# latk/hbetune.rs

Hardware: AMD Instinct MI355X
Metric: GP fit+predict/sec (n=4096,d=8,f64) (higher is better)
Workload: dtype f64; 1 GPU; M: rosenbrock d=8 n=4096 f64, Matern nu=5/2 x constant + white noise; fixed-work fit = 3 L-BFGS runs x 150 lml+gradient evaluations + K^-1, then predict mean+variance at m=1600; evals_per_fit=450, n_not_pd=0, m_candidates=1600, parallelism=replicas x1 (independent fits per GPU, no collective)

## Files before the change

csrc/dag_plan.hpp:

```cpp
#pragma once
#include <algorithm>
#include <cstdint>
#include <cstdio>
#include <queue>
#include <string>
#include <vector>

#include "engine.hpp"

namespace hbegp {

inline int dag_split_point(int lo, int hi) { return lo + (hi - lo) / 2; }

struct DagPlan {
  std::vector<DagTask> tasks;
  std::vector<int> totals;
  double gflop = 0;
  double gflop_lauum = 0;
  int n_lauum = 0;
  int n_leaf = 0;
  double sim_us = 0;
  double crit_us = 0;
};

struct DagGate {
  int cnt = -1, val = 0;
};

struct DagCosts {
  double leaf = 28.5 + 4.0;
  double overhead = 1.5 + 4.0;
  double per128_big = 7.9;
  double per128_small = 3.9;
  double per128_big128 = 15.0;
  double per128_chain = 1.5;
};

class DagBuilder {
 public:
  DagBuilder(int bk, int small_h, int nwg = 0, bool fine = true) : bk_(bk), small_h_(small_h), nwg_(nwg), fine_(fine) {}

  void set_rl(int group, int near, bool lauum_split = true, bool chain32 = true) {
    rl_group_ = std::max(1, group); rl_near_ = std::max(1, near); rl_lauum_split_ = lauum_split; rl_chain32_ = chain32;
  }
  void set_rl_progressive(bool on) { rl_prog_ = on; }
  DagPlan build(int blo, int bhi, bool lauum = false, bool rl = false) {
    plan_ = DagPlan();
    top_lo_ = blo; top_hi_ = bhi;
    if (rl && blo == 0) {
      lauum_split_ = rl_lauum_split_;
      build_rl(bhi, lauum);
    } else {
      const Sub root = rec(blo, bhi, nullptr);
      if (lauum && blo == 0) build_lauum(bhi, root);
    }
    if (plan_.totals.size() >= 0xffff) plan_.tasks.clear();
    for (int tot : plan_.totals)
      if (tot > 0xffff) plan_.tasks.clear();
    if (nwg_ > 0 && !plan_.tasks.empty()) order();
    return plan_;
  }

 private:
  static constexpr int crit_rows_ = 1;
  int bk_, small_h_, nwg_;
  bool fine_;
  int rl_group_ = 32, rl_near_ = 1;
  bool rl_lauum_split_ = true;
  bool big128_ = false;
  bool big128_acc_ = false;
  bool rl_prog_ = false;
  bool rl_chain32_ = true;
  DagPlan plan_;
  DagCosts cost_;

  int new_counter() {
    plan_.totals.push_back(0);
    return (int)plan_.totals.size() - 1;
  }
  void push(DagTask t, const std::vector<DagGate>& waits, int sig0, int sig1, double cost_us, int sig2 = -1) {
// ... 91 lines not shown
      std::stable_sort(tiles.begin() + row_begin, tiles.end(), [](const Tile& a, const Tile& b) {
        auto wt = [](int kind) { return kind == DAG_GEMM_128x128 ? 4 : (kind == DAG_GEMM_128x64 ? 2 : 1); };
        const long wa = (long)(a.kb - a.ka) * wt(a.kind), wb = (long)(b.kb - b.ka) * wt(b.kind);
        return wa > wb;
      });
    }
    return tiles;
  }
  DagTask make(const Op& op, const Tile& tl, double* cost_us) {
    DagTask t{};
    t.kind = (uint16_t)tl.kind;
    t.flags = op.flags;
    t.row0 = tl.row0; t.col0 = tl.col0;
    t.kbeg = tl.ka / bk_ * bk_;
    t.kend = (tl.kb + bk_ - 1) / bk_ * bk_;
    *cost_us = cost_.overhead + (t.kend - t.kbeg) / 128.0 * (tl.kind == DAG_GEMM_128x128 ? cost_.per128_big128 : (tl.kind == DAG_GEMM_128x64 ? cost_.per128_big : (tl.kind == DAG_GEMM_32x64 ? cost_.per128_chain : cost_.per128_small)));
    return t;
  }
  static int count_row(const std::vector<Tile>& tiles, int bi) {
    int c = 0;
    for (const Tile& t : tiles) c += t.bi == bi;
    return c;
  }

  int top_lo_ = 0, top_hi_ = 0, top_mid_ = -1;
  DagGate top_right_all_;
  DagGate top_left_all_;
  bool lauum_split_ = false;
  struct Sub {
    int lo = 0, hi = 0;
    std::vector<DagGate> rowfin;
    DagGate all;
  };
  typedef std::vector<DagGate> RowGates;

  Sub rec(int lo, int hi, const RowGates* gate) {
    Sub out;
    out.lo = lo; out.hi = hi;
    auto gate_of = [&](int i) { return (gate && i < (int)gate->size()) ? (*gate)[i] : DagGate(); };
    if (hi - lo == 1) {
      DagTask t{};
      t.kind = DAG_LEAF;
      t.row0 = lo;
      const int c = new_counter();
      push(t, {gate_of(lo)}, c, -1, cost_.leaf);
      plan_.n_leaf++;
      out.rowfin.assign(1, DagGate{c, 1});
      out.all = DagGate{c, 1};
      return out;
    }
    const int mid = dag_split_point(lo, hi);
    const bool small = std::max(mid - lo, hi - mid) <= small_h_;
    const Sub left = rec(lo, mid, gate);
    double cu = 0;
    Op t{};
    t.flags = DAGF_BBUF | DAGF_CBUF;
    t.r0 = mid; t.r1 = hi; t.c0 = lo; t.c1 = mid; t.k0 = lo; t.k1 = mid; t.klim = 1; t.tri_b = true; t.crit = 1;
    const std::vector<Tile> tt = tiles_of(t, small);
    RowGates trow(hi);
    for (int i = mid; i < hi; ++i) trow[i] = DagGate{new_counter(), count_row(tt, i)};
// ... 123 lines not shown
      stack.push_back({f.lo, mid});
      stack.push_back({mid, f.hi});
    }
    std::vector<DagGate> leafc(nb);
    std::vector<std::vector<DagGate>> lc(nb, std::vector<DagGate>(nb)), last_upd(nb, std::vector<DagGate>(nb));
    std::vector<std::vector<std::pair<int, int>>> groups(nb);
    for (int j = 0; j < nb; ++j) groups[j] = rl_groups(j, GROUP, NEAR);
    double cu = 0;
    auto single_tile = [&](Op op, int i, int j) { op.r0 = i; op.r1 = i + 1; op.c0 = j; op.c1 = j + 1; return op; };
    for (int k = 0; k < nb; ++k) {
      {
        DagTask t{};
        t.kind = DAG_LEAF;
        t.row0 = k;
        const int c = new_counter();
        push(t, {last_upd[k][k]}, c, -1, cost_.leaf);
        plan_.n_leaf++;
        leafc[k] = DagGate{c, 1};
      }
      for (int i = k + 1; i < nb; ++i) {
        Op t{};
        t.flags = DAGF_BBUF | DAGF_C3;
        t.k0 = k; t.k1 = k + 1; t.klim = 1; t.tri_b = true;
        const std::vector<Tile> tt = tiles_of(single_tile(t, i, k), i - k <= NEAR, rl_chain32_ && i == k + 1);
        const int c = new_counter();
        lc[i][k] = DagGate{c, (int)tt.size()};
        const int nd = node_of[i][k];
        for (const Tile& tl : tt) {
          const DagTask tk = make(t, tl, &cu);
          push(tk, {leafc[k], last_upd[i][k], k > 0 ? lc[i][k - 1] : DagGate()}, c, nodes[nd].lrow[i - nodes[nd].mid], cu);
        }
// ... 155 lines not shown
    const std::vector<Tile> xt = tiles_of(x, small);
    RowGates xrow(hi);
    for (int i = mid; i < hi; ++i) xrow[i] = DagGate{new_counter(), count_row(xt, i)};
    const DagGate xall{new_counter(), (int)xt.size()};
    for (const Tile& tl : xt) {
      const DagTask tk = make(x, tl, &cu);
      push(tk, {fine_ ? right.rowfin[tl.bi - mid] : right.all, uall}, xrow[tl.bi].cnt, xall.cnt, cu);
    }
    out.rowfin.resize(hi - lo);
    for (int j = lo; j < mid; ++j) out.rowfin[j - lo] = left.rowfin[j - lo];
    for (int j = mid; j < hi; ++j) out.rowfin[j - lo] = xrow[j];
    out.all = xall;
    return out;
  }

  void order() {
    const int nt = (int)plan_.tasks.size(), nc = (int)plan_.totals.size();
    std::vector<std::vector<int>> waiters(nc);
    for (int i = 0; i < nt; ++i)
      for (int w = 0; w < plan_.tasks[i].nwait; ++w) waiters[plan_.tasks[i].wcnt[w]].push_back(i);
    std::vector<double> bl(nt, 0.0), blc(nc, 0.0);
    for (int i = nt - 1; i >= 0; --i) {
      const DagTask& t = plan_.tasks[i];
      double tail = 0;
      for (int q = 0; q < DAG_MAXSIG; ++q)
        if (t.sig[q] != DAG_NOSIG) tail = std::max(tail, blc[t.sig[q]]);
      bl[i] = t.cost * 0.1 + tail;
      for (int w = 0; w < t.nwait; ++w) blc[t.wcnt[w]] = std::max(blc[t.wcnt[w]], bl[i]);
    }
    plan_.crit_us = *std::max_element(bl.begin(), bl.end());
    std::vector<int> count(nc, 0), missing(nt, 0);
    typedef std::pair<double, int> Pri;
    std::priority_queue<Pri> ready;
    for (int i = 0; i < nt; ++i) {
      missing[i] = plan_.tasks[i].nwait;
      if (missing[i] == 0) ready.push({bl[i], -i});
    }
    typedef std::pair<double, int> Ev;
    std::priority_queue<Ev, std::vector<Ev>, std::greater<Ev>> running;
    std::vector<DagTask> out;
    out.reserve(nt);
    std::vector<int> out_idx;
    std::vector<double> start(nt, 0.0);
    out_idx.reserve(nt);
    int idle = nwg_;
    double now = 0;
    while ((int)out.size() < nt) {
      while (idle > 0 && !ready.empty()) {
        const int i = -ready.top().second;
        ready.pop();
        out.push_back(plan_.tasks[i]);
        out_idx.push_back(i);
        start[i] = now;
        running.push({now + plan_.tasks[i].cost * 0.1, i});
        --idle;
      }
      if (running.empty()) break;
      const Ev e = running.top();
      running.pop();
      now = e.first;
// ... 40 lines not shown
    t.nwait = 0;
    for (int w = 0; w < DAG_MAXWAIT; ++w) t.wcnt[w] = t.wval[w] = 0;
    for (int w = 0; w < src.nwait; ++w) {
      if (remap[src.wcnt[w]] < 0) continue;
      t.wcnt[t.nwait] = (uint16_t)remap[src.wcnt[w]];
      t.wval[t.nwait] = src.wval[w];
      ++t.nwait;
    }
    out.tasks.push_back(t);
  }
  out.gflop = out.gflop_lauum = full.gflop_lauum;
  out.n_lauum = (int)out.tasks.size();
  out.sim_us = full.sim_us;
  out.crit_us = full.crit_us;
  return out;
}

inline std::string dag_plan_validate(const DagPlan& plan, int nblocks_total) {
  const int nc = (int)plan.totals.size(), nt = (int)plan.tasks.size();
  const int words = (nc + 63) / 64;
  char buf[256];
  std::vector<int> count(nc, 0);
  std::vector<uint64_t> counter_known((size_t)nc * words, 0), cur(words);
  const int nt64 = nblocks_total * 4;
  struct Cell { int writer = -1; std::vector<int> readers; };
  constexpr int NBUF = 8;
  std::vector<Cell> cells[NBUF];
  for (int b = 0; b < NBUF; ++b) cells[b].resize((size_t)nt64 * nt64);
  std::vector<std::vector<uint64_t>> known(nt);
  auto hb = [&](int a, int b) -> bool {
// ... 104 lines not shown
```

csrc/hbegp.cpp:

```cpp
#include "../include/hbegp.h"

#include <hip/hip_runtime_api.h>

#include <algorithm>
#include <atomic>
#include <queue>
#include <cmath>
#include <cstdarg>
#include <cstdio>
#include <cstdlib>
#include <cstring>
#include <functional>
#include <limits>
#include <memory>
#include <mutex>
#include <numeric>
#include <string>
#include <thread>
#include <type_traits>
#include <vector>

#include "dag_plan.hpp"
#include "engine.hpp"
#include "lbfgsb.hpp"
// ... 571 lines not shown
    (*off)[w] = (int)items->size();
    items->insert(items->end(), per[w].begin(), per[w].end());
  }
  (*off)[nwg] = (int)items->size();
  *nwg_out = nwg;
  return true;
}

constexpr int DAG_MAX_VARIANTS = 4;
constexpr int DAG_CROWD_LEVELS = 3;
constexpr int DAG_CROWD_BUSY[DAG_CROWD_LEVELS] = {6, 12, 24};
constexpr int DAG_SHARE_VARIANTS = 2;
constexpr int MAX_DEVS = 64;
struct DagPlanKey {
  int blocks, bk, small_h, nwg, lauum, rl, rl_group, rl_near, lauum_split, chain32, prog, big128;
  auto tie() const { return std::tie(blocks, bk, small_h, nwg, lauum, rl, rl_group, rl_near, lauum_split, chain32, prog, big128); }
  bool operator<(const DagPlanKey& o) const { return tie() < o.tie(); }
};
static std::atomic<int> g_dev_busy[MAX_DEVS];
static std::atomic<int> g_dev_fits[MAX_DEVS];

template <typename T>
struct LooIn {
  int dev;
  hipStream_t s;
  int n, d, np, nu2;
  const T *X, *y, *alpha, *Xinv, *Kinv;
  const EvalParams* P;
};
template <typename T>
static int loo_tail(const LooIn<T>& in, T* mean, T* var, T* lpd, double* loo, double* grad);

template <typename T>
struct Slot {
  int dev = 0;
  hipStream_t stream = nullptr;
  T *Xalt = nullptr, *ldalt = nullptr;
  bool x_captured = false;
  T *W1 = nullptr, *W2 = nullptr, *Kinv[2] = {nullptr, nullptr}, *alpha[2] = {nullptr, nullptr};
  T* W3 = nullptr;
  T *ldiag = nullptr, *wbuf = nullptr;
  double *part_t = nullptr, *part_g = nullptr;
  EvalParams* dP = nullptr;
  EvalOut* dOut = nullptr;
  int* tickets = nullptr;
  unsigned long long* dag_trace = nullptr;
  int* dag_ctrl = nullptr;
  EvalParams* hP = nullptr;
  EvalOut* hOut = nullptr;
  void* small_slab = nullptr;
  size_t small_slab_bytes = 0;
  void* host_slab = nullptr;
  size_t host_slab_bytes = 0;
  hipGraphExec_t graph[DAG_MAX_VARIANTS + 1 + DAG_CROWD_LEVELS + DAG_SHARE_VARIANTS][2][4] = {};
  int best_idx = -1;
  double best_lml = -std::numeric_limits<double>::infinity();
  int best_run = 0, best_eval = 0;
  std::vector<double> best_theta;
  std::vector<double> best_params;
  int last_target = 0;
  int dag_variant = 1;
// ... 43 lines not shown
  int dag_nshare_ = 0;
  int share_hyst_ = SLOT_SHARE_HYSTERESIS;
  int slot_maxeval_ = 0;
  std::vector<int> share_force_;
  std::vector<char> balance_dev_;
  std::unique_ptr<std::atomic<int>[]> slot_running_, slot_done_;
  mutable std::atomic<int> not_alone_{0};
  unsigned long long dag_wait_ticks_ = 200000000ull;
  size_t dag_ctrl_bytes = 0;
  int dag_ctrl_regions_ = 1;
  double dag_gflop = 0;
  bool adhoc_ = false;
  bool small_ = false;
  bool like_fit_ = false;
  bool lazy_ = false;
  std::function<std::shared_ptr<const DagPlan>(int, bool)> plan_for_;
  bool hostio_ = true;
  bool eval_published() const { return hostio_ && !small_; }
  int leaf_dbg_ = 0;

  struct Pooled { int dev; void* p; size_t bytes; };
  std::vector<Pooled> pooled_;
  template <typename U>
  U* palloc(int dev, size_t count) {
    bool fresh = false;
    const size_t bytes = std::max<size_t>(16, sizeof(U) * count);
    void* q = g_pool.get(dev, bytes, &fresh);
    pooled_.push_back({dev, q, bytes});
    return static_cast<U*>(q);
  }

// ... 87 lines not shown
      int cus = 1 << 30;
      for (int dev : c->devs) {
        hipDeviceProp_t prop;
        HIPCHECK(hipGetDeviceProperties(&prop, dev));
        cus = std::min(cus, std::max(1, prop.multiProcessorCount));
      }
      const int forced = env_int("HBEGP_DAG_WG", 0);
      auto share_of = [&](int busy) {
        const int share = busy <= 1 ? cus : std::max(8, (cus * 112 / 100 / busy + 4) / 8 * 8);
        return forced > 0 ? forced : std::max(1, std::min(cus, share));
      };
      dag_lauum_ = env_int("HBEGP_DAG_LAUUM", 1) != 0;
      dag_rl_ = env_int("HBEGP_DAG_RL", np / NB <= 80 ? 1 : 0) != 0;
      static std::mutex cache_mu;
      static std::map<DagPlanKey, std::shared_ptr<const DagPlan>> cache;
      plan_for_ = [this](int nwg, bool lauum) {
        const DagPlanKey key = {np / NB, dag_stage_depth(is_f32), env_int("HBEGP_DAG_SMALLH", dag_rl_ ? 4 : 8), nwg, lauum, dag_rl_,
                                env_int("HBEGP_DAG_RL_GROUP", 32), env_int("HBEGP_DAG_RL_NEAR", 1),
                                env_int("HBEGP_DAG_LAUUM_SPLIT", n_slots <= 1 ? 1 : 0),
                                env_int("HBEGP_DAG_CHAIN32", 1),
                                env_int("HBEGP_DAG_PROG", np / NB <= DAG_PROG_MAX_BLOCKS ? 1 : 0),
                                env_int("HBEGP_DAG_BIG128", ((n_slots >= 2 && np / NB >= 32) || np / NB >= 64) ? 2 : 0)};
        std::shared_ptr<const DagPlan> cached;
        {
          std::lock_guard<std::mutex> lk(cache_mu);
          auto it = cache.find(key);
          if (it != cache.end()) cached = it->second;
        }
        if (!cached) {
          DagBuilder builder(key.bk, key.small_h, key.nwg);
          builder.set_rl(key.rl_group, key.rl_near, key.lauum_split != 0, key.chain32 != 0);
          builder.set_rl_progressive(key.prog != 0);
          builder.set_big128(key.big128 != 0, key.big128 >= 2);
          cached = std::make_shared<const DagPlan>(builder.build(0, np / NB, lauum, dag_rl_));
          std::lock_guard<std::mutex> lk(cache_mu);
          if (cache.size() > 256) cache.clear();
          cache[key] = cached;
        }
        return cached;
      };
      const int nvar = std::min(n_slots, DAG_MAX_VARIANTS);
      dag_nwg = share_of(n_slots);
      auto plan_for = [this](int nwg) { return plan_for_(nwg, dag_lauum_); };
      std::shared_ptr<const DagPlan> cached = plan_for(dag_nwg);
      if (cached->tasks.empty() && dag_rl_) {
        dag_rl_ = false;
        cached = plan_for(dag_nwg);
      }
      const DagPlan& plan = *cached;
      if (plan.tasks.empty()) dag_ = dag_lauum_ = false;
      if (dag_ && env_int("HBEGP_DAG_VALIDATE", 0)) {
        const std::string why = dag_plan_validate(plan, np / NB);
        if (!why.empty()) throw std::runtime_error("task queue of the factorisation is unsound: " + why);
      }
      if (dag_) {
        dag_ntasks = (int)plan.tasks.size();
        dag_nwg = std::min(dag_nwg, dag_ntasks);
        dag_gflop = plan.gflop;
// ... 23 lines not shown
          share_force_.resize(n_slots, SLOT_SHARE_EVEN);
        }
        share_hyst_ = std::max(0, env_int("HBEGP_RUN_BALANCE_HYST", SLOT_SHARE_HYSTERESIS));
        dag_nshare_ = (adapt && n_slots > 1 && (env_int("HBEGP_RUN_BALANCE", np / NB >= SLOT_SHARE_MIN_BLOCKS ? 1 : 0) != 0 || !share_force_.empty())) ? DAG_SHARE_VARIANTS : 0;
        if (dag_nshare_) {
          balance_dev_.assign(c->devs.size(), 0);
          slot_running_.reset(new std::atomic<int>[c->devs.size() * n_slots]);
          slot_done_.reset(new std::atomic<int>[c->devs.size() * n_slots]);
          for (size_t i = 0; i < c->devs.size() * n_slots; ++i) { slot_running_[i].store(0); slot_done_[i].store(0); }
        }
        dag_var.assign(nvar + 1 + dag_ncrowd_ + dag_nshare_, DagVariant());
        for (int v = 1; v <= nvar + dag_ncrowd_ + dag_nshare_; ++v) {
          DagVariant& var = dag_var[v];
          std::shared_ptr<const DagPlan> pv = cached;
          var.nwg = dag_nwg;
          if (v != nvar && adapt) {
            if (v > nvar + dag_ncrowd_) {
              var.nwg = std::min(share_wg[v - nvar - dag_ncrowd_ - 1], dag_ntasks);
            } else {
              const int busy = v < nvar ? v : DAG_CROWD_BUSY[v - nvar - 1];
              var.nwg = std::min(share_of(busy), dag_ntasks);
              if (v > nvar) var.nwg = std::min(var.nwg, dag_nwg);
            }
            pv = plan_for(var.nwg);
            if (pv->tasks.size() != plan.tasks.size()) { pv = cached; var.nwg = dag_nwg; }
          }
          var.host_tasks = pv->tasks;
          var.tasks.assign(c->devs.size(), nullptr);
          for (size_t di = 0; di < c->devs.size(); ++di) {
            HIPCHECK(hipSetDevice(c->devs[di]));
            var.tasks[di] = palloc<DagTask>(c->devs[di], pv->tasks.size());
            HIPCHECK(hipMemcpyAsync(var.tasks[di], var.host_tasks.data(), sizeof(DagTask) * var.host_tasks.size(), hipMemcpyHostToDevice, slots[di][0].stream));
          }
          if (lazy_ && dag_lauum_) {
            const int wg_p1 = lazy_wg(var.nwg, 1), wg_kinv = lazy_wg(var.nwg, 2);
            const std::shared_ptr<const DagPlan> p1 = plan_for_(wg_p1, false);
            const DagPlan kv = dag_plan_kinv_only(*pv);
            if (p1->tasks.empty() || kv.tasks.empty() || p1->totals.size() > plan.totals.size() || kv.totals.size() > plan.totals.size()) {
              throw std::runtime_error("task queues of a two-phase evaluation could not be derived from the plan");
            } else {
              if (env_int("HBEGP_DAG_VALIDATE", 0)) {
                std::string why = dag_plan_validate(*p1, np / NB);
                if (why.empty()) why = dag_plan_validate(kv, np / NB);
                if (!why.empty()) throw std::runtime_error("task queue of a two-phase evaluation is unsound: " + why);
              }
              var.host_tasks_p1 = p1->tasks;
              var.host_tasks_kinv = kv.tasks;
              var.ntasks_p1 = (int)p1->tasks.size();
              var.ntasks_kinv = (int)kv.tasks.size();
              var.nwg_p1 = std::min(wg_p1, var.ntasks_p1);
              var.nwg_kinv = std::min(wg_kinv, var.ntasks_kinv);
              var.tasks_p1.assign(c->devs.size(), nullptr);
// ... 40 lines not shown
        if (build_sched(g, sc.tile, &off, &items, &nwg)) {
          sc.nwg = nwg;
          sc.d_off = palloc<int>(s.dev, off.size());
          sc.d_items = palloc<unsigned>(s.dev, items.size());
          HIPCHECK(hipMemcpyAsync(sc.d_off, off.data(), sizeof(int) * off.size(), hipMemcpyHostToDevice, s.stream));
          HIPCHECK(hipMemcpyAsync(sc.d_items, items.data(), sizeof(unsigned) * items.size(), hipMemcpyHostToDevice, s.stream));
          HIPCHECK(hipStreamSynchronize(s.stream));
        }
        scheds[di].push_back(sc);
      };
      eval_gemms(s, s.Kinv[0], record, [](int) {}, [] {});
    }
  }
  ~Problem() override { release(); }

  void release() {
    for (size_t di = 0; di < slots.size(); ++di) {
      (void)hipSetDevice(ctx->devs[di]);
      for (auto& s : slots[di]) {
        if (s.stream) (void)hipStreamSynchronize(s.stream);
        for (int v = 0; v <= DAG_MAX_VARIANTS + DAG_CROWD_LEVELS + DAG_SHARE_VARIANTS; ++v)
          for (int a = 0; a < 2; ++a)
            for (int b = 0; b < 4; ++b)
              if (s.graph[v][a][b]) (void)hipGraphExecDestroy(s.graph[v][a][b]);
        const size_t nnb = sizeof(T) * (size_t)np * np;
        g_pool.put(s.dev, s.W1, nnb); g_pool.put(s.dev, s.W2, nnb); g_pool.put(s.dev, s.W3, nnb);
        for (int b = 0; b < 2; ++b) g_pool.put(s.dev, s.Kinv[b], nnb);
        g_pool.put(s.dev, s.small_slab, s.small_slab_bytes);
        g_host_pool.put(s.host_slab, s.host_slab_bytes);
        g_stream_pool.put(s.dev, s.stream);
      }
// ... 359 lines not shown
          enqueue_eval(s, di, target, mode, nullptr);
        } catch (...) {
          (void)hipStreamEndCapture(s.stream, &gr);
          throw;
        }
        HIPCHECK(hipStreamEndCapture(s.stream, &gr));
        HIPCHECK(hipGraphInstantiate(&ge, gr, nullptr, nullptr, 0));
        HIPCHECK(hipGraphDestroy(gr));
      }
      HIPCHECK(hipGraphLaunch(ge, s.stream));
    } else {
      enqueue_eval(s, di, target, mode, nullptr);
    }
    s.published = eval_published();
    wait_eval(s, t_launch, mode);
    s.last_target = target;
    const int p = d + 2;
    if (s.hOut->info < 0) {
      dag_report_timeout(s);
      throw HipError{hipErrorLaunchTimeOut, "factorisation task queue: a dependency wait exceeded its bound", __LINE__};
    }
    if (s.hOut->info != 0) {
      if (mode != EVAL_GRAD_ONLY) *lml = -std::numeric_limits<double>::infinity();
      if (grad) for (int j = 0; j < p; ++j) grad[j] = 0.0;
      return HBEGP_NOT_PD;
    }
    double lml_kept = s.hOut->lml;
    if (mode == EVAL_GRAD_ONLY) lml = &lml_kept;
    if (!(s.hOut->done & 1) || (want_grad && !(s.hOut->done & 2)))
      throw HipError{hipErrorLaunchFailure, "evaluation: the lml/gradient kernels did not run", __LINE__};
// ... 3589 lines not shown
  DagPlan plan = builder.build(0, nblocks, which != 1, (fine & 8) != 0);
  if (which == 2) plan = dag_plan_kinv_only(plan);
  const std::string why = plan.tasks.empty() ? std::string("no tasks") : dag_plan_validate(plan, nblocks);
  *ntasks = (int)plan.tasks.size();
  if (tasks)
    for (int i = 0; i < std::min(cap, (int)plan.tasks.size()); ++i) {
      const DagTask& t = plan.tasks[i];
      const int v[6] = {t.kind, t.flags, t.row0, t.col0, t.kbeg, t.kend};
      memcpy(tasks + (size_t)6 * i, v, sizeof v);
    }
  if (err && errlen > 0) snprintf(err, (size_t)errlen, "%s", why.c_str());
  return why.empty() ? HBEGP_OK : fail(HBEGP_EINVAL, "%s", why.c_str());
  GUARD_END
}

int hbegp_debug_lbfgs_replay(int n, const double* x0, const double* lo, const double* hi, int maxeval, int memory, int fixed_work,
                             int count, const double* f, const double* g, double* requested, int* n_requested) {
  if (n < 1 || n > LBFGS_MAXN || count < 0 || !x0 || !lo || !hi || !requested || !n_requested || (count > 0 && (!f || !g)))
    return fail(HBEGP_EINVAL, "bad argument");
  GUARD_BEGIN
  return lbfgs_replay_impl(n, x0, lo, hi, maxeval, memory, fixed_work, count, f, g, requested, nullptr, nullptr, nullptr, n_requested);
  GUARD_END
}

int hbegp_debug_dag_plan(int nblocks, int bk, int small_h, int nwg, int fine, int* ntasks, int* ncounters, int* nleaf,
                         double* gflop, double* crit_us, double* sim_us, char* err, int errlen) {
  if (nblocks < 1 || (bk != 16 && bk != 32) || small_h < 0 || nwg < 0) return fail(HBEGP_EINVAL, "bad argument");
  GUARD_BEGIN
  DagBuilder builder(bk, small_h, nwg, (fine & 1) != 0);
  builder.set_rl_progressive((fine & 16) != 0);
// ... 48 lines not shown
```

hbetune_rs_amd/_lib.py:

```python
import ctypes as C
import os

import numpy as np

HERE = os.path.dirname(os.path.abspath(__file__))
LIB_PATH = os.environ.get("HBEGP_LIB") or os.path.join(HERE, "libhbegp.so")

OK, NOT_PD, ALL_FAILED = 0, 1, 2
EINVAL, EHIP, ENODEV, ENOMEM = -1, -2, -3, -4
PATHS_MAX_FEATURES, PATHS_MAX_PATHS = 16384, 1024
CEI_MAX_CONSTRAINTS = 8
MES_MAX_SAMPLES = 1024
EHVI_ND_MAX_BOXES = 1048576
STATS_MAX_RUNS = 16


class HbegpError(RuntimeError):
    def __init__(self, code, msg):
        super().__init__(f"hbegp error {code}: {msg}")
        self.code = code


class FitOptions(C.Structure):

# ... 154 lines not shown
    "hbegp_debug_lcei_phases": (C.c_int, [C.c_int, _dp]),
    "hbegp_debug_mes_phases": (C.c_int, [C.c_int, _dp]),
    "hbegp_debug_cb_phases": (C.c_int, [C.c_int, _dp]),
    "hbegp_debug_pool_poisoned": (C.c_int, [C.POINTER(C.c_longlong), C.POINTER(C.c_longlong)]),
    "hbegp_model_info": (C.c_int, [_vp, _ip, _ip, _ip, _dp, _dp]),
    "hbegp_model_get_f64": (C.c_int, [_vp, _dp, _dp, _dp]),
    "hbegp_model_get_f32": (C.c_int, [_vp, _dp, _fp, _fp]),
    "hbegp_model_debug_params": (C.c_int, [_vp, _dp]),
    "hbegp_model_retain": (None, [_vp]),
    "hbegp_model_release": (None, [_vp]),
    "hbegp_debug_lbfgs_replay": (C.c_int, [C.c_int, _dp, _dp, _dp, C.c_int, C.c_int, C.c_int, C.c_int, _dp, _dp, _dp, _ip]),
    "hbegp_last_fit_stats": (C.c_int, [C.POINTER(FitStats)]),
    "hbegp_debug_lbfgs_decisions": (C.c_int, [C.c_int, _dp, _dp, _dp, C.c_int, C.c_int, C.c_int, C.c_int, _dp, _dp, _dp, _ip, _ip, _ip, _ip]),
    "hbegp_debug_dag_queues": (C.c_int, [C.c_int, C.c_int, C.c_int, C.c_int, C.c_int, C.c_int, C.c_int, _ip, _ip, C.c_int, C.c_char_p,
                                         C.c_int]),
    "hbegp_debug_slot_shares": (C.c_int, [C.c_int, _ip, _ip, _ip, C.c_int, _ip, C.c_int, C.c_int, _ip, _ip]),
    "hbegp_debug_fits_in_flight": (C.c_int, [C.c_int]),
    "hbegp_debug_dag_plan": (C.c_int, [C.c_int, C.c_int, C.c_int, C.c_int, C.c_int, _ip, _ip, _ip, _dp, _dp, _dp, C.c_char_p,
                                       C.c_int]),
    "hbegp_minimize_by_gradient": (C.c_double, [OBJECTIVE_FN, _vp, _dp, _dp, _dp, C.c_int, C.c_int]),
    "hbegp_problem_create_rv_f64": (C.c_int, [_vp, _dp, _dp, _dp, C.c_int, C.c_int, C.c_double, C.c_int, C.POINTER(_vp)]),
    "hbegp_problem_create_rv_f32": (C.c_int, [_vp, _fp, _fp, _dp, C.c_int, C.c_int, C.c_double, C.c_int, C.POINTER(_vp)]),
    "hbegp_fit_rv_f64": (C.c_int, [_vp, _dp, _dp, _dp, C.c_int, C.c_int, C.c_double, _dp, _dp, _dp, _dp, C.c_int,
                                   C.POINTER(FitOptions), _dp, _dp, C.POINTER(_vp)]),
    "hbegp_fit_rv_f32": (C.c_int, [_vp, _fp, _fp, _dp, C.c_int, C.c_int, C.c_double, _dp, _dp, _dp, _dp, C.c_int,
                                   C.POINTER(FitOptions), _dp, _dp, C.POINTER(_vp)]),
    "hbegp_fit_loo_rv_f64": (C.c_int, [_vp, _dp, _dp, _dp, C.c_int, C.c_int, C.c_double, _dp, _dp, _dp, _dp, C.c_int,
                                       C.POINTER(FitOptions), _dp, _dp, C.POINTER(_vp)]),
    "hbegp_fit_loo_rv_f32": (C.c_int, [_vp, _fp, _fp, _dp, C.c_int, C.c_int, C.c_double, _dp, _dp, _dp, _dp, C.c_int,
                                       C.POINTER(FitOptions), _dp, _dp, C.POINTER(_vp)]),
# ... 59 lines not shown
```

include/hbegp.h:

```cpp
#ifndef HBEGP_H
#define HBEGP_H

#include <stddef.h>

#ifdef __cplusplus
extern "C" {
#endif

#define HBEGP_VERSION 200

enum {
  HBEGP_OK = 0,
  HBEGP_NOT_PD = 1,
  HBEGP_ALL_FAILED = 2,
  HBEGP_EINVAL = -1,
  HBEGP_EHIP = -2,
  HBEGP_ENODEV = -3,
  HBEGP_ENOMEM = -4
};

typedef struct hbegp_ctx hbegp_ctx;
typedef struct hbegp_problem hbegp_problem;
typedef struct hbegp_model hbegp_model;

// ... 252 lines not shown
int hbegp_model_debug_params(hbegp_model* model, double* out);

int hbegp_debug_dag_plan(int nblocks, int bk, int small_h, int nwg, int fine, int* ntasks, int* ncounters, int* nleaf,
                         double* gflop, double* crit_us, double* sim_us, char* err, int errlen);

int hbegp_debug_lbfgs_replay(int n, const double* x0, const double* lo, const double* hi, int maxeval, int memory, int fixed_work,
                             int count, const double* f, const double* g, double* requested, int* n_requested);

int hbegp_debug_lbfgs_decisions(int n, const double* x0, const double* lo, const double* hi, int maxeval, int memory, int fixed_work,
                                int count, const double* f, const double* g, double* requested, int* trial, int* accepted, int* took,
                                int* n_requested);

int hbegp_debug_dag_queues(int nblocks, int bk, int small_h, int nwg, int fine, int big128, int which, int* ntasks, int* tasks, int cap,
                           char* err, int errlen);

int hbegp_debug_slot_shares(int n_slots, const int* running, const int* done, const int* maxeval, int hysteresis, int* share, int even_wg,
                            int cus, int* lead_wg, int* lag_wg);
int hbegp_debug_fits_in_flight(int device_id);

int hbegp_debug_pool_poisoned(long long* blocks, long long* bytes);
int hbegp_debug_posterior_phases(int enable, double* phase_ms);
int hbegp_debug_batch_select_phases(int enable, double* phase_ms);
int hbegp_debug_kg_phases(int enable, double* phase_ms);
int hbegp_debug_nei_phases(int enable, double* phase_ms);
int hbegp_debug_ehvi_phases(int enable, double* phase_ms);
int hbegp_debug_ehvi_nd_phases(int enable, double* phase_ms);
int hbegp_debug_ehvi_boxes(const double* front, int P, int n_obj, const double* ref, int* thr_count, double* thr, int thr_cap,
                           int* n_boxes, int* boxes, int box_cap);
int hbegp_debug_cei_phases(int enable, double* phase_ms);
int hbegp_debug_lcei_phases(int enable, double* phase_ms);
// ... 29 lines not shown
```

Measured before the change: 1.969 fit+predict/s.

## Recalibrate DAG task cost model and order lead-share queues for even worker count

Adds a per-kind fixed plus per-k cost model with a separate signalling cost, used for plans of at least 32 blocks. The old costs are kept for small plans. When there are two or more slots, the lead-share variant's task queue is ordered by simulating the even worker count instead of its own, so priority ordering better matches the workgroups that actually run it. It also adds an optional level-ordering mode, a replay simulator, and per-evaluation trace capture for debugging. The aim is a queue order with less stall on dependencies, at the risk of worse ordering if the cost model is off.

```diff
diff --git a/csrc/dag_plan.hpp b/csrc/dag_plan.hpp
--- a/csrc/dag_plan.hpp
+++ b/csrc/dag_plan.hpp
@@ -23,22 +23,46 @@
   double crit_us = 0;
 };
 
+constexpr int DAG_ORDER_BY_LEVEL = -1;
+
+constexpr int DAG_ORDER_MIN_BLOCKS = 32;
+inline int dag_default_order_wg(int queue, int share, int nwg, int even_wg, int nblocks, int n_slots) {
+  (void)queue;
+  if (n_slots < 2 || nblocks < DAG_ORDER_MIN_BLOCKS) return 0;
+  if (share == 2 && even_wg > 0 && even_wg < nwg) return even_wg;
+  return 0;
+}
+
 struct DagGate {
   int cnt = -1, val = 0;
 };
 
 struct DagCosts {
-  double leaf = 28.5 + 4.0;
-  double overhead = 1.5 + 4.0;
-  double per128_big = 7.9;
-  double per128_small = 3.9;
+  static DagCosts round2() {
+    DagCosts c;
+    c.signal = 4.0; c.leaf = 28.5;
+    c.fixed_small = c.fixed_big = c.fixed_big128 = c.fixed_chain = 1.5; c.acc_big128 = 0.0;
+    c.per128_big = 7.9; c.per128_small = 3.9; c.per128_big128 = c.per128_big128_km = 15.0; c.per128_chain = 1.5;
+    return c;
+  }
+  double signal = 1.1;
+  double leaf = 26.3;
+  double fixed_small = 3.5;
+  double fixed_big = 4.0;
+  double fixed_big128 = 4.2;
+  double acc_big128 = 1.8;
+  double fixed_chain = 3.2;
+  double per128_big = 8.1;
+  double per128_small = 4.0;
   double per128_big128 = 15.0;
-  double per128_chain = 1.5;
+  double per128_big128_km = 15.0;
+  double per128_chain = 2.5;
 };
 
 class DagBuilder {
  public:
-  DagBuilder(int bk, int small_h, int nwg = 0, bool fine = true) : bk_(bk), small_h_(small_h), nwg_(nwg), fine_(fine) {}
+  DagBuilder(int bk, int small_h, int nwg = 0, bool fine = true, int order_wg = 0)
+      : bk_(bk), small_h_(small_h), nwg_(nwg), order_wg_(order_wg == 0 ? nwg : order_wg), fine_(fine) {}
 
   void set_rl(int group, int near, bool lauum_split = true, bool chain32 = true) {
     rl_group_ = std::max(1, group); rl_near_ = std::max(1, near); rl_lauum_split_ = lauum_split; rl_chain32_ = chain32;
@@ -46,6 +70,7 @@
   void set_rl_progressive(bool on) { rl_prog_ = on; }
   DagPlan build(int blo, int bhi, bool lauum = false, bool rl = false) {
     plan_ = DagPlan();
+    cost_ = bhi - blo >= DAG_ORDER_MIN_BLOCKS ? DagCosts() : DagCosts::round2();
     top_lo_ = blo; top_hi_ = bhi;
     if (rl && blo == 0) {
       lauum_split_ = rl_lauum_split_;
@@ -57,13 +82,16 @@
     if (plan_.totals.size() >= 0xffff) plan_.tasks.clear();
     for (int tot : plan_.totals)
       if (tot > 0xffff) plan_.tasks.clear();
-    if (nwg_ > 0 && !plan_.tasks.empty()) order();
+    if (nwg_ > 0 && !plan_.tasks.empty()) {
+      if (order_wg_ < 0) order_by_level();
+      else order();
+    }
     return plan_;
   }
 
  private:
   static constexpr int crit_rows_ = 1;
-  int bk_, small_h_, nwg_;
+  int bk_, small_h_, nwg_, order_wg_;
   bool fine_;
   int rl_group_ = 32, rl_near_ = 1;
   bool rl_lauum_split_ = true;
@@ -185,7 +213,12 @@
     t.row0 = tl.row0; t.col0 = tl.col0;
     t.kbeg = tl.ka / bk_ * bk_;
     t.kend = (tl.kb + bk_ - 1) / bk_ * bk_;
-    *cost_us = cost_.overhead + (t.kend - t.kbeg) / 128.0 * (tl.kind == DAG_GEMM_128x128 ? cost_.per128_big128 : (tl.kind == DAG_GEMM_128x64 ? cost_.per128_big : (tl.kind == DAG_GEMM_32x64 ? cost_.per128_chain : cost_.per128_small)));
+    const bool km = (op.flags & (DAGF_AKM | DAGF_BKM)) != 0;
+    double fixed = cost_.fixed_small, rate = cost_.per128_small;
+    if (tl.kind == DAG_GEMM_128x128) { fixed = cost_.fixed_big128 + ((op.flags & DAGF_ACC) ? cost_.acc_big128 : 0.0); rate = km ? cost_.per128_big128_km : cost_.per128_big128; }
+    if (tl.kind == DAG_GEMM_128x64) { fixed = cost_.fixed_big; rate = cost_.per128_big; }
+    if (tl.kind == DAG_GEMM_32x64) { fixed = cost_.fixed_chain; rate = cost_.per128_chain; }
+    *cost_us = cost_.signal + fixed + (t.kend - t.kbeg) / 128.0 * rate;
     return t;
   }
   static int count_row(const std::vector<Tile>& tiles, int bi) {
@@ -214,7 +247,7 @@
       t.kind = DAG_LEAF;
       t.row0 = lo;
       const int c = new_counter();
-      push(t, {gate_of(lo)}, c, -1, cost_.leaf);
+      push(t, {gate_of(lo)}, c, -1, cost_.leaf + cost_.signal);
       plan_.n_leaf++;
       out.rowfin.assign(1, DagGate{c, 1});
       out.all = DagGate{c, 1};
@@ -368,7 +401,7 @@
         t.kind = DAG_LEAF;
         t.row0 = k;
         const int c = new_counter();
-        push(t, {last_upd[k][k]}, c, -1, cost_.leaf);
+        push(t, {last_upd[k][k]}, c, -1, cost_.leaf + cost_.signal);
         plan_.n_leaf++;
         leafc[k] = DagGate{c, 1};
       }
@@ -554,11 +587,8 @@
     return out;
   }
 
-  void order() {
+  std::vector<double> bottom_levels() {
     const int nt = (int)plan_.tasks.size(), nc = (int)plan_.totals.size();
-    std::vector<std::vector<int>> waiters(nc);
-    for (int i = 0; i < nt; ++i)
-      for (int w = 0; w < plan_.tasks[i].nwait; ++w) waiters[plan_.tasks[i].wcnt[w]].push_back(i);
     std::vector<double> bl(nt, 0.0), blc(nc, 0.0);
     for (int i = nt - 1; i >= 0; --i) {
       const DagTask& t = plan_.tasks[i];
@@ -569,6 +599,17 @@
       for (int w = 0; w < t.nwait; ++w) blc[t.wcnt[w]] = std::max(blc[t.wcnt[w]], bl[i]);
     }
     plan_.crit_us = *std::max_element(bl.begin(), bl.end());
+    return bl;
+  }
+
+  void order_by_level();
+
+  void order() {
+    const int nt = (int)plan_.tasks.size(), nc = (int)plan_.totals.size();
+    std::vector<std::vector<int>> waiters(nc);
+    for (int i = 0; i < nt; ++i)
+      for (int w = 0; w < plan_.tasks[i].nwait; ++w) waiters[plan_.tasks[i].wcnt[w]].push_back(i);
+    const std::vector<double> bl = bottom_levels();
     std::vector<int> count(nc, 0), missing(nt, 0);
     typedef std::pair<double, int> Pri;
     std::priority_queue<Pri> ready;
@@ -583,7 +624,7 @@
     std::vector<int> out_idx;
     std::vector<double> start(nt, 0.0);
     out_idx.reserve(nt);
-    int idle = nwg_;
+    int idle = order_wg_;
     double now = 0;
     while ((int)out.size() < nt) {
       while (idle > 0 && !ready.empty()) {
@@ -654,6 +695,67 @@
   out.sim_us = full.sim_us;
   out.crit_us = full.crit_us;
   return out;
+}
+
+struct DagReplay {
+  double makespan_us = 0, wait_us = 0, busy_us = 0;
+};
+inline DagReplay dag_plan_replay(const DagPlan& plan, int workers) {
+  DagReplay out;
+  const int nt = (int)plan.tasks.size(), nc = (int)plan.totals.size();
+  if (workers < 1 || nt == 0) return out;
+  std::vector<double> done(nc, 0.0);
+  std::priority_queue<double, std::vector<double>, std::greater<double>> free_at;
+  for (int w = 0; w < std::min(workers, nt); ++w) free_at.push(0.0);
+  for (int i = 0; i < nt; ++i) {
+    const DagTask& t = plan.tasks[i];
+    const double claimed = free_at.top();
+    free_at.pop();
+    double start = claimed;
+    for (int w = 0; w < t.nwait; ++w) start = std::max(start, done[t.wcnt[w]]);
+    const double end = start + t.cost * 0.1;
+    for (int q = 0; q < DAG_MAXSIG; ++q)
+      if (t.sig[q] != DAG_NOSIG) done[t.sig[q]] = std::max(done[t.sig[q]], end);
+    out.wait_us += start - claimed;
+    out.busy_us += t.cost * 0.1;
+    out.makespan_us = std::max(out.makespan_us, end);
+    free_at.push(end);
+  }
+  return out;
+}
+
+inline void DagBuilder::order_by_level() {
+  const int nt = (int)plan_.tasks.size(), nc = (int)plan_.totals.size();
+  std::vector<std::vector<int>> waiters(nc);
+  for (int i = 0; i < nt; ++i)
+    for (int w = 0; w < plan_.tasks[i].nwait; ++w) waiters[plan_.tasks[i].wcnt[w]].push_back(i);
+  const std::vector<double> bl = bottom_levels();
+  std::vector<int> count(nc, 0), missing(nt, 0);
+  typedef std::pair<double, int> Pri;
+  std::priority_queue<Pri> ready;
+  for (int i = 0; i < nt; ++i) {
+    missing[i] = plan_.tasks[i].nwait;
+    if (missing[i] == 0) ready.push({bl[i], -i});
+  }
+  std::vector<DagTask> out;
+  out.reserve(nt);
+  while (!ready.empty()) {
+    const int i = -ready.top().second;
+    ready.pop();
+    out.push_back(plan_.tasks[i]);
+    const DagTask& t = plan_.tasks[i];
+    for (int q = 0; q < DAG_MAXSIG; ++q) {
+      if (t.sig[q] == DAG_NOSIG) continue;
+      const int c = t.sig[q];
+      if (++count[c] == plan_.totals[c])
+        for (int wtr : waiters[c])
+          if (--missing[wtr] == 0) ready.push({bl[wtr], -wtr});
+    }
+  }
+  if ((int)out.size() == nt) {
+    plan_.tasks.swap(out);
+    plan_.sim_us = dag_plan_replay(plan_, nwg_).makespan_us;
+  }
 }
 
 inline std::string dag_plan_validate(const DagPlan& plan, int nblocks_total) {
diff --git a/csrc/hbegp.cpp b/csrc/hbegp.cpp
--- a/csrc/hbegp.cpp
+++ b/csrc/hbegp.cpp
@@ -609,7 +609,8 @@
 constexpr int MAX_DEVS = 64;
 struct DagPlanKey {
   int blocks, bk, small_h, nwg, lauum, rl, rl_group, rl_near, lauum_split, chain32, prog, big128;
-  auto tie() const { return std::tie(blocks, bk, small_h, nwg, lauum, rl, rl_group, rl_near, lauum_split, chain32, prog, big128); }
+  int order_wg;
+  auto tie() const { return std::tie(blocks, bk, small_h, nwg, lauum, rl, rl_group, rl_near, lauum_split, chain32, prog, big128, order_wg); }
   bool operator<(const DagPlanKey& o) const { return tie() < o.tie(); }
 };
 static std::atomic<int> g_dev_busy[MAX_DEVS];
@@ -640,6 +641,8 @@
   EvalOut* dOut = nullptr;
   int* tickets = nullptr;
   unsigned long long* dag_trace = nullptr;
+  struct KeptTrace { unsigned long long seq; int part, variant, nwg; std::vector<unsigned long long> stamps; };
+  std::vector<KeptTrace> kept_traces;
   int* dag_ctrl = nullptr;
   EvalParams* hP = nullptr;
   EvalOut* hOut = nullptr;
@@ -713,7 +716,7 @@
   bool small_ = false;
   bool like_fit_ = false;
   bool lazy_ = false;
-  std::function<std::shared_ptr<const DagPlan>(int, bool)> plan_for_;
+  std::function<std::shared_ptr<const DagPlan>(int, bool, int)> plan_for_;
   bool hostio_ = true;
   bool eval_published() const { return hostio_ && !small_; }
   int leaf_dbg_ = 0;
@@ -831,13 +834,14 @@
       dag_rl_ = env_int("HBEGP_DAG_RL", np / NB <= 80 ? 1 : 0) != 0;
       static std::mutex cache_mu;
       static std::map<DagPlanKey, std::shared_ptr<const DagPlan>> cache;
-      plan_for_ = [this](int nwg, bool lauum) {
+      plan_for_ = [this](int nwg, bool lauum, int order_wg) {
         const DagPlanKey key = {np / NB, dag_stage_depth(is_f32), env_int("HBEGP_DAG_SMALLH", dag_rl_ ? 4 : 8), nwg, lauum, dag_rl_,
                                 env_int("HBEGP_DAG_RL_GROUP", 32), env_int("HBEGP_DAG_RL_NEAR", 1),
                                 env_int("HBEGP_DAG_LAUUM_SPLIT", n_slots <= 1 ? 1 : 0),
                                 env_int("HBEGP_DAG_CHAIN32", 1),
                                 env_int("HBEGP_DAG_PROG", np / NB <= DAG_PROG_MAX_BLOCKS ? 1 : 0),
-                                env_int("HBEGP_DAG_BIG128", ((n_slots >= 2 && np / NB >= 32) || np / NB >= 64) ? 2 : 0)};
+                                env_int("HBEGP_DAG_BIG128", ((n_slots >= 2 && np / NB >= 32) || np / NB >= 64) ? 2 : 0),
+                                (order_wg == nwg || nwg <= 0) ? 0 : order_wg};
         std::shared_ptr<const DagPlan> cached;
         {
           std::lock_guard<std::mutex> lk(cache_mu);
@@ -845,11 +849,15 @@
           if (it != cache.end()) cached = it->second;
         }
         if (!cached) {
-          DagBuilder builder(key.bk, key.small_h, key.nwg);
+          DagBuilder builder(key.bk, key.small_h, key.nwg, true, key.order_wg);
           builder.set_rl(key.rl_group, key.rl_near, key.lauum_split != 0, key.chain32 != 0);
           builder.set_rl_progressive(key.prog != 0);
           builder.set_big128(key.big128 != 0, key.big128 >= 2);
           cached = std::make_shared<const DagPlan>(builder.build(0, np / NB, lauum, dag_rl_));
+          if (key.order_wg != 0 && !cached->tasks.empty()) {
+            const std::string why = dag_plan_validate(*cached, np / NB);
+            if (!why.empty()) throw std::runtime_error("task queue ordered for another worker count is unsound: " + why);
+          }
           std::lock_guard<std::mutex> lk(cache_mu);
           if (cache.size() > 256) cache.clear();
           cache[key] = cached;
@@ -858,7 +866,14 @@
       };
       const int nvar = std::min(n_slots, DAG_MAX_VARIANTS);
       dag_nwg = share_of(n_slots);
-      auto plan_for = [this](int nwg) { return plan_for_(nwg, dag_lauum_); };
+      auto order_wg_for = [this](int queue, int share, int nwg) {
+        const char* name = share == SLOT_SHARE_LEAD ? "HBEGP_DAG_ORDER_WG_LEAD"
+                           : (share == SLOT_SHARE_LAG ? "HBEGP_DAG_ORDER_WG_LAG"
+                              : (queue == 1 ? "HBEGP_DAG_ORDER_WG_P1" : (queue == 2 ? "HBEGP_DAG_ORDER_WG_KINV" : "HBEGP_DAG_ORDER_WG")));
+        const int forced = env_int(name, 0);
+        return forced != 0 ? std::max(forced, DAG_ORDER_BY_LEVEL) : dag_default_order_wg(queue, share, nwg, dag_nwg, np / NB, n_slots);
+      };
+      auto plan_for = [this, order_wg_for](int nwg, int share = SLOT_SHARE_EVEN) { return plan_for_(nwg, dag_lauum_, order_wg_for(0, share, nwg)); };
       std::shared_ptr<const DagPlan> cached = plan_for(dag_nwg);
       if (cached->tasks.empty() && dag_rl_) {
         dag_rl_ = false;
@@ -912,6 +927,7 @@
           DagVariant& var = dag_var[v];
           std::shared_ptr<const DagPlan> pv = cached;
           var.nwg = dag_nwg;
+          const int share = v > nvar + dag_ncrowd_ ? (v == nvar + dag_ncrowd_ + 1 ? SLOT_SHARE_LEAD : SLOT_SHARE_LAG) : SLOT_SHARE_EVEN;
           if (v != nvar && adapt) {
             if (v > nvar + dag_ncrowd_) {
               var.nwg = std::min(share_wg[v - nvar - dag_ncrowd_ - 1], dag_ntasks);
@@ -920,7 +936,7 @@
               var.nwg = std::min(share_of(busy), dag_ntasks);
               if (v > nvar) var.nwg = std::min(var.nwg, dag_nwg);
             }
-            pv = plan_for(var.nwg);
+            pv = plan_for(var.nwg, share);
             if (pv->tasks.size() != plan.tasks.size()) { pv = cached; var.nwg = dag_nwg; }
           }
           var.host_tasks = pv->tasks;
@@ -932,8 +948,10 @@
           }
           if (lazy_ && dag_lauum_) {
             const int wg_p1 = lazy_wg(var.nwg, 1), wg_kinv = lazy_wg(var.nwg, 2);
-            const std::shared_ptr<const DagPlan> p1 = plan_for_(wg_p1, false);
-            const DagPlan kv = dag_plan_kinv_only(*pv);
+            const std::shared_ptr<const DagPlan> p1 = plan_for_(wg_p1, false, order_wg_for(1, share, wg_p1));
+            const int order_kinv = order_wg_for(2, share, wg_kinv);
+            const std::shared_ptr<const DagPlan> pk = order_kinv == 0 ? pv : plan_for_(var.nwg, true, order_kinv);
+            const DagPlan kv = dag_plan_kinv_only(*pk);
             if (p1->tasks.empty() || kv.tasks.empty() || p1->totals.size() > plan.totals.size() || kv.totals.size() > plan.totals.size()) {
               throw std::runtime_error("task queues of a two-phase evaluation could not be derived from the plan");
             } else {
@@ -1004,7 +1022,45 @@
   }
   ~Problem() override { release(); }
 
+  void keep_fit_trace(Slot<T>& s, int mode) {
+    static const char* range = getenv("HBEGP_DAG_TRACE_EVALS");
+    int a = 0, b = 0;
+    if (!range || !dag_ || !s.dag_trace || sscanf(range, "%d:%d", &a, &b) != 2 || s.seq < (unsigned long long)std::max(a, 0) || s.seq >= (unsigned long long)std::max(b, 0)) return;
+    const int part = !(lazy_ && dag_lauum_) ? 0 : (mode == EVAL_LML_ONLY ? 1 : (mode == EVAL_GRAD_ONLY ? 2 : 0));
+    const DagVariant& var = dag_var[s.dag_variant];
+    typename Slot<T>::KeptTrace k;
+    k.seq = s.seq; k.part = part; k.variant = s.dag_variant;
+    k.nwg = part == 1 ? var.nwg_p1 : (part == 2 ? var.nwg_kinv : var.nwg);
+    k.stamps.resize((size_t)5 * (part == 1 ? var.ntasks_p1 : (part == 2 ? var.ntasks_kinv : dag_ntasks)));
+    HIPCHECK(hipMemcpyAsync(k.stamps.data(), s.dag_trace, sizeof(unsigned long long) * k.stamps.size(), hipMemcpyDeviceToHost, s.stream));
+    HIPCHECK(hipStreamSynchronize(s.stream));
+    s.kept_traces.push_back(std::move(k));
+  }
+  void write_fit_traces() {
+    const char* prefix = getenv("HBEGP_DAG_TRACE");
+    for (size_t di = 0; prefix && di < slots.size(); ++di)
+      for (size_t si = 0; si < slots[di].size(); ++si)
+        for (const auto& k : slots[di][si].kept_traces) {
+          if (k.variant < 0 || k.variant >= (int)dag_var.size()) continue;
+          const DagVariant& var = dag_var[k.variant];
+          const std::vector<DagTask>& tasks = k.part == 1 ? var.host_tasks_p1 : (k.part == 2 ? var.host_tasks_kinv : var.host_tasks);
+          char name[512];
+          snprintf(name, sizeof name, "%s.s%zu.e%llu.p%d", prefix, si, k.seq, k.part);
+          FILE* f = fopen(name, "w");
+          if (!f) continue;
+          fprintf(f, "# slot %zu evaluation %llu part %d variant %d share %d nwg %d tasks %zu\n", si, k.seq, k.part, k.variant, share_of_variant(k.variant), k.nwg, tasks.size());
+          for (size_t i = 0; i < tasks.size() && 5 * i + 4 < k.stamps.size(); ++i) {
+            const DagTask& t = tasks[i];
+            const unsigned long long* tr = k.stamps.data() + 5 * i;
+            fprintf(f, "%zu %d %d %d %d %d %llu %llu %llu %llu %llu %llu %d\n", i, t.kind, t.row0, t.col0, t.kend - t.kbeg, t.nwait, tr[0], tr[1], tr[2], tr[3], tr[4] >> 32,
+                    tr[4] & 0xffffffffull, t.flags);
+          }
+          fclose(f);
+        }
+  }
+
   void release() {
+    write_fit_traces();
     for (size_t di = 0; di < slots.size(); ++di) {
       (void)hipSetDevice(ctx->devs[di]);
       for (auto& s : slots[di]) {
@@ -1394,6 +1450,7 @@
     }
     s.published = eval_published();
     wait_eval(s, t_launch, mode);
+    if (s.dag_trace) keep_fit_trace(s, mode);
     s.last_target = target;
     const int p = d + 2;
     if (s.hOut->info < 0) {
@@ -5013,6 +5070,43 @@
   GUARD_END
 }
 
+int hbegp_debug_dag_replay(int nblocks, int bk, int small_h, int nwg, int order_wg, int fine, int big128, int which, int workers,
+                           int* ntasks, int* tasks, int cap, double* out, char* err, int errlen) {
+  if (nblocks < 1 || (bk != 16 && bk != 32) || small_h < 0 || nwg < 1 || which < 0 || which > 2 || !ntasks || workers < 0)
+    return fail(HBEGP_EINVAL, "bad argument");
+  GUARD_BEGIN
+  DagBuilder builder(bk, small_h, nwg, (fine & 1) != 0, order_wg);
+  builder.set_rl_progressive((fine & 16) != 0);
+  builder.set_big128(big128 != 0, big128 >= 2);
+  builder.set_rl(32, 1, (fine & 32) == 0, true);
+  DagPlan plan = builder.build(0, nblocks, which != 1, (fine & 8) != 0);
+  if (which == 2) plan = dag_plan_kinv_only(plan);
+  const std::string why = plan.tasks.empty() ? std::string("no tasks") : dag_plan_validate(plan, nblocks);
+  *ntasks = (int)plan.tasks.size();
+  if (tasks)
+    for (int i = 0; i < std::min(cap, (int)plan.tasks.size()); ++i) {
+      const DagTask& t = plan.tasks[i];
+      int* v = tasks + (size_t)18 * i;
+      v[0] = t.kind; v[1] = t.flags; v[2] = t.row0; v[3] = t.col0; v[4] = t.kbeg; v[5] = t.kend; v[6] = t.nwait;
+      for (int w = 0; w < DAG_MAXWAIT; ++w) { v[7 + w] = w < t.nwait ? t.wcnt[w] : 0; v[11 + w] = w < t.nwait ? t.wval[w] : 0; }
+      for (int q = 0; q < DAG_MAXSIG; ++q) v[15 + q] = t.sig[q];
+    }
+  if (out) {
+    const DagReplay r = workers > 0 ? dag_plan_replay(plan, workers) : DagReplay();
+    double acc128 = 0;
+    for (const DagTask& t : plan.tasks)
+      if (t.kind == DAG_GEMM_128x128 && (t.flags & DAGF_ACC)) acc128 += t.cost * 0.1;
+    out[0] = r.makespan_us; out[1] = r.wait_us; out[2] = r.busy_us; out[3] = plan.sim_us; out[4] = plan.crit_us; out[5] = acc128;
+  }
+  if (err && errlen > 0) snprintf(err, (size_t)errlen, "%s", why.c_str());
+  return why.empty() ? HBEGP_OK : fail(HBEGP_EINVAL, "%s", why.c_str());
+  GUARD_END
+}
+
+int hbegp_debug_dag_order_wg(int queue, int share, int nwg, int even_wg, int nblocks, int n_slots) {
+  return dag_default_order_wg(queue, share, nwg, even_wg, nblocks, n_slots);
+}
+
 int hbegp_debug_lbfgs_replay(int n, const double* x0, const double* lo, const double* hi, int maxeval, int memory, int fixed_work,
                              int count, const double* f, const double* g, double* requested, int* n_requested) {
   if (n < 1 || n > LBFGS_MAXN || count < 0 || !x0 || !lo || !hi || !requested || !n_requested || (count > 0 && (!f || !g)))
diff --git a/hbetune_rs_amd/_lib.py b/hbetune_rs_amd/_lib.py
--- a/hbetune_rs_amd/_lib.py
+++ b/hbetune_rs_amd/_lib.py
@@ -192,6 +192,9 @@
     "hbegp_debug_lbfgs_decisions": (C.c_int, [C.c_int, _dp, _dp, _dp, C.c_int, C.c_int, C.c_int, C.c_int, _dp, _dp, _dp, _ip, _ip, _ip, _ip]),
     "hbegp_debug_dag_queues": (C.c_int, [C.c_int, C.c_int, C.c_int, C.c_int, C.c_int, C.c_int, C.c_int, _ip, _ip, C.c_int, C.c_char_p,
                                          C.c_int]),
+    "hbegp_debug_dag_replay": (C.c_int, [C.c_int, C.c_int, C.c_int, C.c_int, C.c_int, C.c_int, C.c_int, C.c_int, C.c_int, _ip, _ip,
+                                         C.c_int, _dp, C.c_char_p, C.c_int]),
+    "hbegp_debug_dag_order_wg": (C.c_int, [C.c_int, C.c_int, C.c_int, C.c_int, C.c_int, C.c_int]),
     "hbegp_debug_slot_shares": (C.c_int, [C.c_int, _ip, _ip, _ip, C.c_int, _ip, C.c_int, C.c_int, _ip, _ip]),
     "hbegp_debug_fits_in_flight": (C.c_int, [C.c_int]),
     "hbegp_debug_dag_plan": (C.c_int, [C.c_int, C.c_int, C.c_int, C.c_int, C.c_int, _ip, _ip, _ip, _dp, _dp, _dp, C.c_char_p,
diff --git a/include/hbegp.h b/include/hbegp.h
--- a/include/hbegp.h
+++ b/include/hbegp.h
@@ -290,6 +290,10 @@
 int hbegp_debug_dag_queues(int nblocks, int bk, int small_h, int nwg, int fine, int big128, int which, int* ntasks, int* tasks, int cap,
                            char* err, int errlen);
 
+int hbegp_debug_dag_replay(int nblocks, int bk, int small_h, int nwg, int order_wg, int fine, int big128, int which, int workers,
+                           int* ntasks, int* tasks, int cap, double* out, char* err, int errlen);
+int hbegp_debug_dag_order_wg(int queue, int share, int nwg, int even_wg, int nblocks, int n_slots);
+
 int hbegp_debug_slot_shares(int n_slots, const int* running, const int* done, const int* maxeval, int hysteresis, int* share, int even_wg,
                             int cus, int* lead_wg, int* lag_wg);
 int hbegp_debug_fits_in_flight(int device_id);
```

New measurement: 1.995 fit+predict/s, median of 6. +1.3%, better.
